# GStreamer/gst-plugins-rs

Hardware: AMD Instinct MI355X
Metric: 4K RGBA frames/sec through hsvfilter+colorlut at 1 GPU; % HBM roofline (higher is better)
Workload: dtype u8

## Files before the change

gst-plugins-rs_amd/csrc/autopick.hpp:

```cpp
#pragma once
#include <cstddef>

namespace mi355 {

constexpr unsigned kProbeMin = 64, kProbeMax = 1024;
constexpr double kDecisive = 2.0;
constexpr double kRegimeChange = 1.25;

struct AutoPolicy {
  unsigned calls = 0, since_probe = 0, probe_period = kProbeMin;
  bool table = false;
  double t_compute = 0.0, t_table = 0.0;
  size_t vec = 0;
  int pending_kind = -1;
  size_t pending_vec = 0;
  unsigned pending_call = 0;
  bool pending_probe = false, pending_discard = false;
  unsigned learn = 0;
  bool probe_second = false;
  bool table_unavailable = false;
  double hysteresis = 0.03;
  double hysteresis_back = -1.0;
  bool smooth = false;
  bool last_probe = false;
// ... 55 lines not shown
    D.discard = (A.learn & 1) == 0;
    D.probe = true;
    if (A.pending_kind < 0) A.learn++;
  } else {
    D.kind = A.table ? 1 : 0;
    bool warming = false;
    if (A.probe_second) {
      A.probe_second = false;
      D.kind ^= 1;
      D.probe = true;
    } else if (++A.since_probe >= A.probe_period && A.pending_kind < 0) {
      A.since_probe = 0;
      A.probe_second = true;
      D.kind ^= 1;
      warming = true;
    }
    if (warming) { A.calls++; return D; }
  }
  D.measure = A.pending_kind < 0 && (D.probe || (A.calls % auto_sample_every(n_vec)) == 0);
  A.calls++;
  return D;
}

inline void auto_sampled(AutoPolicy &A, const AutoDecision &D, size_t n_vec) {
  A.pending_kind = D.kind;
  A.pending_call = A.calls;
  A.pending_vec = n_vec;
  A.pending_probe = D.probe && A.t_compute > 0.0 && A.t_table > 0.0;
  A.pending_discard = D.discard;
}

inline void auto_give_up_table(AutoPolicy &A) {
  A.table_unavailable = true;
  A.learn = 4;
  A.table = false;
}

}
```

gst-plugins-rs_amd/csrc/colorlut_kernels.hip:

```cpp
#include "internal.hpp"
#include "hsv_device.hpp"
#include "exact_math.hpp"

#include <cmath>
#include <cstring>
#include <map>
#include <memory>
#include <mutex>
#include <vector>

namespace mi355 {

struct LutK {
  float scale[3];
  float offset[3];
  int size;
};


__device__ __forceinline__ uint32_t floor_idx(float x, uint32_t max_idx) {
  const float f = floorf(x);
  uint32_t i = (f > 0.0f) ? ((f >= 4294967040.0f) ? 0xffffffffu : (uint32_t)f) : 0u;
  return i < max_idx ? i : max_idx;
}
// ... 825 lines not shown
  __shared__ uint32_t s_strip[4][512];
  s_spread[threadIdx.x] = spread3(threadIdx.x);
  __syncthreads();
  auto index = [&](uint32_t p) -> uint32_t { return s_spread[p & 0xffu] | (s_spread[(p >> 8) & 0xffu] << 1) | (s_spread[(p >> 16) & 0xffu] << 2); };
  const unsigned wave = threadIdx.x >> 6, lane = threadIdx.x & 63;
  uint32_t *x = s_strip[wave];
  const unsigned frame = blockIdx.x / tiles_per_frame, t = blockIdx.x - frame * tiles_per_frame;
  const u32x4_t *s4 = (const u32x4_t *)srcs.p[frame];
  u32x4_t *d4 = (u32x4_t *)dsts.p[frame];
  auto wave_sync = [] {
    __builtin_amdgcn_fence(__ATOMIC_ACQ_REL, "wavefront");
    __builtin_amdgcn_wave_barrier();
  };
  constexpr unsigned RPL = 64 / TW4;
  const unsigned sub = lane / TW4, g = lane % TW4;
  const unsigned tx = t % n_cols, ty = t / n_cols;
  const unsigned col = tx * TW4 + g;
  const unsigned r0 = ty * (8 * RPL) + wave * (2 * RPL) + sub, r1 = r0 + RPL;
  const bool ok0 = col < w4 && r0 < rows, ok1 = col < w4 && r1 < rows;
  const size_t i0 = (size_t)r0 * w4 + col, i1 = (size_t)r1 * w4 + col;
  u32x4_t p = {0, 0, 0, 0}, q = {0, 0, 0, 0};
  if (ok0) p = __builtin_nontemporal_load(s4 + i0);
  if (ok1) q = __builtin_nontemporal_load(s4 + i1);
  *(u32x4_t *)(x + lane * 4) = p;
  *(u32x4_t *)(x + 256 + lane * 4) = q;
  wave_sync();
  uint32_t px[8], o[8];
#pragma unroll
  for (int j = 0; j < 8; j++) px[j] = x[j * 64 + lane];
#pragma unroll
  for (int j = 0; j < 8; j++) o[j] = table[index(px[j])];
#pragma unroll
  for (int j = 0; j < 8; j++) x[j * 64 + lane] = (o[j] & 0x00ffffffu) | (px[j] & 0xff000000u);
  wave_sync();
  const u32x4_t r0v = *(u32x4_t *)(x + lane * 4), r1v = *(u32x4_t *)(x + 256 + lane * 4);
  if (ok0) __builtin_nontemporal_store(r0v, d4 + i0);
  if (ok1) __builtin_nontemporal_store(r1v, d4 + i1);
}

void shared_table_release(mi355_ctx *ctx, std::shared_ptr<void> *ref);
void lut_release(mi355_ctx *ctx) {
  for (int i = 0; i < 2; i++) {
    shared_table_release(ctx, &ctx->lut.table_ref[i]);
    if (ctx->lut.pick[i].ev0) (void)hipEventDestroy(ctx->lut.pick[i].ev0);
    if (ctx->lut.pick[i].ev1) (void)hipEventDestroy(ctx->lut.pick[i].ev1);
  }
// ... 713 lines not shown
  MultiFramePtrs s{}, d{};
  for (int f = 0; f < n_frames; f++) {
    if (!srcs[f] || !dsts[f] || (uintptr_t)srcs[f] % 16 != 0 || (uintptr_t)dsts[f] % 16 != 0) return MI355_ERR_UNSUPPORTED;
    s.p[f] = srcs[f];
    d.p[f] = dsts[f];
  }
  const unsigned w4 = (unsigned)width / 4;
  if (from_hbm && ctx->lut_variant == 0 && window_multi_applicable(ctx, w4, (size_t)height, n_frames)) {
    ctx->lut.last_kernel = "colorlut_window_kernel";
    return launch_window_table_multi(ctx, stream, table, srcs, dsts, n_frames, w4, (size_t)height);
  }
  ctx->lut.last_kernel = "colorlut_table_tiled_multi_kernel";
  const unsigned pad64 = (w4 + 63) / 64 * 64 - w4, pad32 = (w4 + 31) / 32 * 32 - w4;
  const unsigned tw4 = pad64 <= pad32 ? 64 : 32;
  const unsigned n_cols = (w4 + tw4 - 1) / tw4, rpb = 8 * (64 / tw4);
  const size_t tiles_per_frame = (size_t)n_cols * (((size_t)height + rpb - 1) / rpb);
  const size_t grid = tiles_per_frame * (size_t)n_frames;
  if (grid >= (1u << 31)) return MI355_ERR_UNSUPPORTED;
  if (tw4 == 64) hipLaunchKernelGGL((colorlut_table_tiled_multi_kernel<64>), dim3((unsigned)grid), dim3(256), 0, stream, s, d, w4, (unsigned)height, n_cols, (unsigned)tiles_per_frame, table);
  else hipLaunchKernelGGL((colorlut_table_tiled_multi_kernel<32>), dim3((unsigned)grid), dim3(256), 0, stream, s, d, w4, (unsigned)height, n_cols, (unsigned)tiles_per_frame, table);
  return check_hip(ctx, hipGetLastError(), "colorlut multi-frame table kernel launch");
}

void hsv_table_release(mi355_ctx *ctx) {
  HsvTable &T = ctx->hsv_table;
  shared_table_release(ctx, &T.table_ref);
  if (T.pick.ev0) (void)hipEventDestroy(T.pick.ev0);
  if (T.pick.ev1) (void)hipEventDestroy(T.pick.ev1);
  T = HsvTable{};
}

static int hsv_table_ensure(mi355_ctx *ctx, const PixFmt &fmt, const mi355_hsv_settings &hs) {
  HsvTable &T = ctx->hsv_table;
  if (T.valid && T.bgr == fmt.bgr && same_hs(T.hs, hs)) return MI355_OK;
  T.valid = false;
  T.d_table = nullptr;
  std::string key("H");
  key.push_back((char)('0' + fmt.bgr));
  key.append((const char *)&hs, sizeof(hs));
  int rc = shared_table_acquire(ctx, key, &T.table_ref, &T.d_table, [&](uint32_t *tab) {
    hipLaunchKernelGGL(table_domain_kernel, dim3(kTableEntries / 256), dim3(256), 0, ctx->stream, tab, 1);
    return launch_hsvfilter_compute(ctx, (uint8_t *)tab, 1, 0, 4096, 4096, 4096 * 4, fmt, hs);
  });
  if (rc) { T.table_ref.reset(); T.d_table = nullptr; return rc; }
  T.valid = true;
  T.bgr = fmt.bgr;
// ... 67 lines not shown
```

gst-plugins-rs_amd/csrc/ctx.hip:

```cpp
#include "internal.hpp"
#include <mutex>

#include <cstdio>
#include <cstring>

namespace mi355 {

bool pixfmt_of(int format, PixFmt *out) {
  switch (format) {
    case MI355_FMT_RGBX: *out = {4, 0, 0, 0}; return true;
    case MI355_FMT_RGBA: *out = {4, 0, 0, 1}; return true;
    case MI355_FMT_XRGB: *out = {4, 1, 0, 0}; return true;
    case MI355_FMT_ARGB: *out = {4, 1, 0, 1}; return true;
    case MI355_FMT_BGRX: *out = {4, 0, 1, 0}; return true;
    case MI355_FMT_BGRA: *out = {4, 0, 1, 1}; return true;
    case MI355_FMT_XBGR: *out = {4, 1, 1, 0}; return true;
    case MI355_FMT_ABGR: *out = {4, 1, 1, 1}; return true;
    case MI355_FMT_RGB: *out = {3, 0, 0, 0}; return true;
    case MI355_FMT_BGR: *out = {3, 0, 1, 0}; return true;
    default: return false;
  }
}

int set_error(mi355_ctx *ctx, int status, const std::string &msg) {
// ... 61 lines not shown
}

const char *mi355_status_string(int status) {
  switch (status) {
    case MI355_OK: return "ok";
    case MI355_ERR_INVALID_ARG: return "invalid argument";
    case MI355_ERR_NO_DEVICE: return "no usable gfx950 device";
    case MI355_ERR_HIP: return "HIP runtime error";
    case MI355_ERR_NOT_CONFIGURED: return "element not configured";
    case MI355_ERR_OUT_OF_MEMORY: return "out of device memory";
    case MI355_ERR_UNSUPPORTED: return "unsupported";
    case MI355_ERR_TIMEOUT: return "timeout";
    default: return "unknown status";
  }
}

}

namespace mi355 {
namespace {
struct Written { uintptr_t lo = 0, hi = 0; };
std::mutex g_written_mu;
Written g_written[16][2];
constexpr size_t kOnDieBytes = (size_t)320 << 20;
}

void note_written(int device, const void *p, size_t bytes) {
  if (device < 0 || device >= 16 || !p || !bytes) return;
  std::lock_guard<std::mutex> lk(g_written_mu);
  g_written[device][1] = g_written[device][0];
  g_written[device][0].lo = (uintptr_t)p;
  g_written[device][0].hi = (uintptr_t)p + bytes;
}

void forget_written(int device, const void *p, size_t bytes) {
  if (device < 0 || device >= 16 || !p || !bytes) return;
  std::lock_guard<std::mutex> lk(g_written_mu);
  for (Written &w : g_written[device])
    if (w.hi > w.lo && (uintptr_t)p < w.hi && (uintptr_t)p + bytes > w.lo) w = Written{};
}

bool recently_written(int device, const void *p, size_t bytes) {
  if (device < 0 || device >= 16 || !p || !bytes || bytes > kOnDieBytes) return false;
  std::lock_guard<std::mutex> lk(g_written_mu);
  for (const Written &w : g_written[device])
    if (w.hi > w.lo && (uintptr_t)p >= w.lo && (uintptr_t)p + bytes <= w.hi && w.hi - w.lo <= kOnDieBytes) return true;
  return false;
// ... 81 lines not shown

int mi355_ctx_synchronize(mi355_ctx *ctx) {
  REQUIRE_CTX(ctx);
  BIND_DEVICE(ctx);
  return check_hip(ctx, hipStreamSynchronize(ctx->stream), "hipStreamSynchronize");
}

int mi355_ctx_set_flag(mi355_ctx *ctx, int flag, int value) {
  REQUIRE_CTX(ctx);
  if (flag == MI355_FLAG_FORCE_GENERIC) { ctx->force_generic = value != 0; return MI355_OK; }
  if (flag == MI355_FLAG_LUT_STAGGER && value >= 0 && value <= 4096) { ctx->lut_stagger = value; return MI355_OK; }
  if (flag == MI355_FLAG_LUT_VARIANT && value >= 0 && value <= 9) { ctx->lut_variant = value; return MI355_OK; }
  if (flag == MI355_FLAG_BRICK_TILES_PER_RUN && value >= 0 && value <= 4096) { ctx->brick_tiles_per_run = value; return MI355_OK; }
  if (flag == MI355_FLAG_BRICK_FOLD_AXIS && value >= 0 && value <= 2) { ctx->brick_fold_axis = value; return MI355_OK; }
  if (flag == MI355_FLAG_DSSIM_TRANSLUCENT && (value == 0 || value == 1)) { ctx->dssim_translucent = value; return MI355_OK; }
  if (flag == MI355_FLAG_DSSIM_FAST && (value == 0 || value == 1)) { ctx->dssim_fast = value; return MI355_OK; }
  if (flag == MI355_FLAG_BRICK_PRIO && value >= 0 && value <= 3) { ctx->brick_prio = value; return MI355_OK; }
  if (flag == MI355_FLAG_BRICK_SETS && (value == 0 || value == 32 || value == 48 || value == 64 || value == 512)) { ctx->brick_sets = value; return MI355_OK; }
  if (flag == MI355_FLAG_HSV_TABLE && value >= 0 && value <= 3) { ctx->hsv_table_mode = value; return MI355_OK; }
  if (flag == MI355_FLAG_FUSED_VARIANT && value >= 0 && value <= 1) { ctx->fused_variant = value; return MI355_OK; }
  if (flag == MI355_FLAG_HSV_BLOCKS_PER_CU && value >= 1 && value <= 4096) { ctx->hsv_blocks_per_cu = value; return MI355_OK; }
  if (flag == MI355_FLAG_HRTF_METHOD && value >= 0 && value <= 2) { ctx->hrtf_method = value; return MI355_OK; }
  if (flag == MI355_FLAG_BLOCKHASH_ANY_SIZE && (value == 0 || value == 1)) { ctx->blockhash_any_size = value; return MI355_OK; }
  if (flag == MI355_FLAG_HSV_NT && (value == 0 || value == 1)) { ctx->hsv_nt = value; return MI355_OK; }
  if (flag == MI355_FLAG_WINDOW_ORDER && (value == 0 || value == 1)) { ctx->window_order = value; return MI355_OK; }
  if (flag == MI355_FLAG_WINDOW_STATS && (value == 0 || value == 1)) { ctx->window_stats_on = value != 0; return MI355_OK; }
  if (flag == MI355_FLAG_WINDOW_MIN_STEPS && value >= 0 && value <= 4096) { ctx->window_min_steps = value; return MI355_OK; }
  return set_error(ctx, MI355_ERR_INVALID_ARG, "unknown flag");
}

void *mi355_device_alloc(mi355_ctx *ctx, size_t bytes) {
  if (!ctx) return nullptr;
  if (hipSetDevice(ctx->device) != hipSuccess) return nullptr;
  void *p = nullptr;
  if (check_hip(ctx, hipMalloc(&p, bytes ? bytes : 16), "hipMalloc")) return nullptr;
  return p;
}

int mi355_device_free(mi355_ctx *ctx, void *dptr) {
  REQUIRE_CTX(ctx);
  BIND_DEVICE(ctx);
  return check_hip(ctx, hipFree(dptr), "hipFree");
}

int mi355_memcpy_h2d(mi355_ctx *ctx, void *dptr, const void *host, size_t bytes) {
  REQUIRE_CTX(ctx);
  BIND_DEVICE(ctx);
// ... 592 lines not shown
}

int mi355_issue_streams_round(mi355_ctx *const *ctxs, int n_streams, uint8_t *const *d_src, uint8_t *const *d_dst, int width, int height, int stride,
                              int format, const mi355_hsv_settings *settings) {
  if (!ctxs || !d_src || !d_dst || !settings || n_streams < 0) return MI355_ERR_INVALID_ARG;
  const size_t pitch = (size_t)stride * (size_t)(height > 0 ? height : 0);
  for (int i = 0; i < n_streams; i++) {
    int rc = mi355_hsvfilter_frames_device(ctxs[i], d_src[i], 1, pitch, width, height, stride, format, settings);
    if (rc) return rc;
    rc = mi355_colorlut_frames_device(ctxs[i], d_src[i], pitch, stride, d_dst[i], pitch, stride, 1, width, height, format);
    if (rc) return rc;
  }
  return MI355_OK;
}

int mi355_hsv_colorlut_chain_batches_device(mi355_ctx *ctx, uint8_t *const *d_src, uint8_t *const *d_dst, int n_batches, int n_frames, size_t frame_pitch,
                                            int stride, int width, int height, int format, const mi355_hsv_settings *settings, int lanes) {
  REQUIRE_CTX(ctx);
  if (!d_src || !d_dst || !settings || n_batches < 0 || lanes < 1 || lanes > 2) return set_error(ctx, MI355_ERR_INVALID_ARG, "chain batches: bad argument");
  BIND_DEVICE(ctx);
  int rc = MI355_OK;
  for (int k = 0; k < n_batches && !rc; k++) {
    if (!d_src[k] || !d_dst[k]) { rc = set_error(ctx, MI355_ERR_INVALID_ARG, "chain batches: null batch"); break; }
    rc = mi355_hsvfilter_frames_device(ctx, d_src[k], n_frames, frame_pitch, width, height, stride, format, settings);
    if (!rc) rc = mi355_colorlut_frames_device(ctx, d_src[k], frame_pitch, stride, d_dst[k], frame_pitch, stride, n_frames, width, height, format);
  }
  return rc;
}

int mi355_dssim_compare_frames_device(mi355_ctx *ctx, const mi355_dssim_image *original, const uint8_t *const *d_frames, int n_frames, int stride,
                                      int width, int height, int format, double *dssim) {
  REQUIRE_CTX(ctx);
  int channels = 0;
  int rc = dssim_channels(ctx, format, &channels);
  if (rc) return rc;
  if (!original || !d_frames || !dssim || n_frames < 0 || width <= 0 || height <= 0 || (size_t)stride < (size_t)width * channels)
    return set_error(ctx, MI355_ERR_INVALID_ARG, "dssim: bad frames");
  for (int f = 0; f < n_frames; f++)
    if (!d_frames[f]) return set_error(ctx, MI355_ERR_INVALID_ARG, "dssim: null frame");
  if (n_frames == 0) return MI355_OK;
  BIND_DEVICE(ctx);
  return dssim_compare_frames(ctx, original, d_frames, n_frames, stride, width, height, channels, dssim);
}

int mi355_dssim_compare_frames(mi355_ctx *ctx, const mi355_dssim_image *original, const uint8_t *const *frames, int n_frames, int stride, int width,
                               int height, int format, double *dssim) {
// ... 199 lines not shown
```

gst-plugins-rs_amd/csrc/group.hip:

```cpp
#include "internal.hpp"

#include <chrono>
#include <condition_variable>
#include <algorithm>
#include <cstring>
#include <deque>
#include <mutex>
#include <unordered_map>
#include <vector>

using namespace mi355;

namespace {

struct Desc {
  mi355_ctx *ctx;
  uint8_t *src, *dst;
  int width, height, stride, format;
  mi355_hsv_settings hs;
  const uint32_t *table;
  std::shared_ptr<void> table_ref;
  bool batchable;
  bool fused;
  uint64_t ticket;
// ... 743 lines not shown
    if (!lk.owns_lock()) lk.lock();
    reap.swap(g->dead_refs);
    lk.unlock();
  }
};

void retire_front(mi355_group *g) {
  Batch &b = g->batches.front();
  for (uint64_t t : b.tickets) g->where.erase(t);
  g->events.push_back(b.done);
  if (b.table_ref) g->dead_refs.push_back(std::move(b.table_ref));
  g->batches.pop_front();
}

void retire_done(mi355_group *g) {
  while (!g->batches.empty() && g->batches.front().waiters == 0) {
    if (hipEventQuery(g->batches.front().done) != hipSuccess) { (void)hipGetLastError(); break; }
    retire_front(g);
  }
}

bool same_class(const Desc &a, const Desc &b) {
  return a.batchable && b.batchable && a.fused == b.fused && a.width == b.width && a.height == b.height && a.stride == b.stride && a.format == b.format && a.table == b.table &&
         std::memcmp(&a.hs, &b.hs, sizeof(a.hs)) == 0 && a.ctx->force_generic == b.ctx->force_generic;
}

int flush_locked(mi355_group *g, uint64_t until = 0) {
  bool reached = false;
  while (!g->pending.empty() && !reached) {
    std::vector<Desc> take, keep;
    std::vector<mi355_ctx *> blocked;
    const Desc first = g->pending.front();
    for (const Desc &d : g->pending) {
      bool stream_blocked = false;
      for (mi355_ctx *c : blocked) stream_blocked |= c == d.ctx;
      const bool fits = take.empty() || (!stream_blocked && (int)take.size() < g->max_batch && same_class(first, d));
      if (fits) take.push_back(d);
      else keep.push_back(d);
      if (!stream_blocked) blocked.push_back(d.ctx);
    }
    g->pending.swap(keep);
    PixFmt fmt;
    (void)pixfmt_of(first.format, &fmt);
    hipEvent_t done = take_event(g);
    if (!done) return fail(g, MI355_ERR_HIP, "hipEventCreate");
    int rc = MI355_OK;
    if (first.batchable) {
      uint8_t *srcs[kMultiFrames], *dsts[kMultiFrames];
      for (size_t i = 0; i < take.size(); i++) {
        srcs[i] = take[i].src;
        dsts[i] = take[i].dst;
        if (take[i].ready && hipStreamWaitEvent(g->stream, take[i].ready, 0) != hipSuccess) rc = MI355_ERR_HIP;
      }
      if (!rc && !first.fused) rc = launch_hsvfilter_multi(first.ctx, g->stream, srcs, (int)take.size(), first.width, first.height, fmt, first.hs);
      if (!rc) rc = launch_colorlut_multi(first.ctx, g->stream, first.table, srcs, dsts, (int)take.size(), first.width, first.height, first.fused);
      if (!rc && hipEventRecord(done, g->stream) != hipSuccess) rc = MI355_ERR_HIP;
      g->n_batched_launch_pairs++;
    } else {
      const Desc &d = take[0];
      const size_t pitch = (size_t)d.stride * (size_t)d.height;
      if (!g->batches.empty() && hipStreamWaitEvent(d.ctx->stream, g->batches.back().done, 0) != hipSuccess) rc = MI355_ERR_HIP;
      if (!rc && d.fused) rc = launch_hsv_colorlut(d.ctx, d.src, pitch, d.stride, d.dst, pitch, d.stride, 1, d.width, d.height, d.hs);
      if (!rc && !d.fused) rc = launch_hsvfilter(d.ctx, d.src, 1, pitch, d.width, d.height, d.stride, fmt, d.hs);
      if (!rc && !d.fused) rc = launch_colorlut(d.ctx, d.src, pitch, d.stride, d.dst, pitch, d.stride, 1, d.width, d.height, d.format);
      if (!rc && hipEventRecord(done, d.ctx->stream) != hipSuccess) rc = MI355_ERR_HIP;
      if (!rc && hipStreamWaitEvent(g->stream, done, 0) != hipSuccess) rc = MI355_ERR_HIP;
      if (rc && rc != MI355_ERR_HIP) g->last_error = d.ctx->last_error;
      g->n_single++;
    }
    for (const Desc &d : take)
      if (d.ready) g->events.push_back(d.ready);
    if (rc) {
      (void)hipGetLastError();
      g->events.push_back(done);
      if (g->failed.size() > 65536) g->failed.clear();
      for (const Desc &d : take) g->failed[d.ticket] = rc;
      if (g->last_error.empty()) g->last_error = "group launch failed";
      return rc;
// ... 575 lines not shown
```

gst-plugins-rs_amd/csrc/hsv_device.hpp:

```cpp
#pragma once
#include "internal.hpp"
#include "exact_math.hpp"

namespace mi355 {

struct HsvK {
  float hue_shift, sat_mul, sat_off, val_mul, val_off;
};


template <bool FAST>
__device__ __forceinline__ void hsv_from_rgb(float r8, float g8, float b8, float &hue, float &sat,
                                             float &val) {
  if constexpr (FAST) {
    const float r = div255_u8(r8), g = div255_u8(g8), b = div255_u8(b8);
    const float value = fmaxf(fmaxf(r, g), b);
    const float minv = fminf(fminf(r, g), b);
    const float chroma = value - minv;
    const bool is_r = (r == value);
    const bool is_g = (g == value);
    const float na = is_r ? g : (is_g ? b : r);
    const float nb = is_r ? b : (is_g ? r : g);
    const float add = is_r ? 0.0f : (is_g ? 2.0f : 4.0f);
    const float q = div_rcp_refine(na - nb, fmaxf(chroma, 1e-30f));
    float h = 60.0f * (add + q);
// ... 288 lines not shown
    r = (r >= 360.0f) ? r - 360.0f : r;
    return __builtin_copysignf(r, t);
  }
  return fmodf(t, 360.0f);
}
template <int RPOS, int GPOS, int BPOS, int NPOS>
__device__ __forceinline__ void hsvfilter_px2_generic(uint32_t &p0, uint32_t &p1, const HsvK &k, const HsvLds *lds) {
  f2 h2, sat, value;
  hsv_from_rgb_pair_fast<RPOS, GPOS, BPOS, 1>(p0, p1, h2, sat, value, lds);
  uint32_t *px[2] = {&p0, &p1};
#pragma unroll
  for (int j = 0; j < 2; j++) {
    float h = hsv_fmod360_any((j ? h2.y : h2.x) + k.hue_shift);
    if (h < 0.0f) h += 360.0f;
    const float s = fminf(fmaxf(k.sat_mul * (j ? sat.y : sat.x) + k.sat_off, 0.0f), 1.0f);
    const float v = fminf(fmaxf(k.val_mul * (j ? value.y : value.x) + k.val_off, 0.0f), 1.0f);
    uint32_t r, g, b;
    hsv_to_rgb_generic(h, s, v, r, g, b);
    const uint32_t keep = *px[j] & (0xffu << (8 * NPOS));
    *px[j] = keep | (r << (8 * RPOS)) | (g << (8 * GPOS)) | (b << (8 * BPOS));
  }
}

inline int hsv_variant_for(const mi355_hsv_settings &s, bool force_generic, bool allow_wide = false) {
  const float a = fabsf(s.hue_shift);
  const bool narrow = (s.hue_shift == 0.0f) || (a >= 1e-30f && a <= 360.0f);
  const bool wide = allow_wide && a > 360.0f && a <= 4194304.0f;
  if (!(narrow || wide) || force_generic) return -1;
  const bool sv_ident = s.saturation_mul == 1.0f && s.saturation_off == 0.0f && s.value_mul == 1.0f && s.value_off == 0.0f;
  if (wide) return 8 | (s.hue_shift < 0.0f ? 1 : 0) | (sv_ident ? 4 : 0);
  const int shift = s.hue_shift == 0.0f ? HSV_SHIFT_ZERO : (s.hue_shift > 0.0f ? HSV_SHIFT_POS : HSV_SHIFT_NEG);
  return shift | (sv_ident ? 4 : 0);
}

}
```

gst-plugins-rs_amd/csrc/hsv_kernels.hip:

```cpp
#include "internal.hpp"
#include "exact_math.hpp"
#include "hsv_device.hpp"

namespace mi355 {


template <int VARIANT, int RPOS, int GPOS, int BPOS, int NPOS>
__device__ __forceinline__ void hsvfilter_quad(uint32_t &a, uint32_t &b, uint32_t &c, uint32_t &d, const HsvK &k, const HsvLds *lds) {
  if constexpr (VARIANT >= 0) {
    hsvfilter_px2_lds<RPOS, GPOS, BPOS, NPOS, hsv_shift_of(VARIANT), hsv_sv_ident_of(VARIANT)>(a, b, k, lds);
    hsvfilter_px2_lds<RPOS, GPOS, BPOS, NPOS, hsv_shift_of(VARIANT), hsv_sv_ident_of(VARIANT)>(c, d, k, lds);
  } else {
    hsvfilter_px2_generic<RPOS, GPOS, BPOS, NPOS>(a, b, k, lds);
    hsvfilter_px2_generic<RPOS, GPOS, BPOS, NPOS>(c, d, k, lds);
  }
}

template <int VARIANT, int FIRST, bool BGR>
__global__ __launch_bounds__(256) void hsvfilter_flat_kernel(uint4 *__restrict__ data, size_t n_vec,
                                                             HsvK k, int nt) {
  constexpr int RPOS = FIRST + (BGR ? 2 : 0), GPOS = FIRST + 1, BPOS = FIRST + (BGR ? 0 : 2);
  constexpr int NPOS = FIRST == 0 ? 3 : 0;
  __shared__ HsvLds lds;
  hsv_lds_fill<RPOS, GPOS, BPOS, NPOS>(&lds);
  __syncthreads();
  const size_t stride = (size_t)gridDim.x * blockDim.x;
  if (nt) {
    typedef uint32_t u32x4_t __attribute__((ext_vector_type(4)));
    u32x4_t *d4 = (u32x4_t *)data;
    for (size_t i = (size_t)blockIdx.x * blockDim.x + threadIdx.x; i < n_vec; i += stride) {
      const u32x4_t v = __builtin_nontemporal_load(d4 + i);
      uint4 p = {v.x, v.y, v.z, v.w};
      hsvfilter_quad<VARIANT, RPOS, GPOS, BPOS, NPOS>(p.x, p.y, p.z, p.w, k, &lds);
      const u32x4_t o = {p.x, p.y, p.z, p.w};
      __builtin_nontemporal_store(o, d4 + i);
    }
    return;
  }
  for (size_t i = (size_t)blockIdx.x * blockDim.x + threadIdx.x; i < n_vec; i += stride) {
// ... 162 lines not shown
    const size_t r = i - f * per_frame;
    const size_t row = r / (size_t)width;
    const size_t col = r - row * (size_t)width;
    uint8_t *px = data + f * frame_pitch + row * (size_t)stride + col * (size_t)pixel_stride + first;
    const uint32_t c0 = px[0], c1 = px[1], c2 = px[2];
    const uint32_t p = bgr ? (c2 | (c1 << 8) | (c0 << 16)) : (c0 | (c1 << 8) | (c2 << 16));
    const uint32_t o = hsvfilter_px<FAST, 0, 1, 2, 3>(p, k, sel_tab);
    const uint8_t orr = (uint8_t)(o & 0xff), og = (uint8_t)((o >> 8) & 0xff), ob = (uint8_t)((o >> 16) & 0xff);
    px[0] = bgr ? ob : orr;
    px[1] = og;
    px[2] = bgr ? orr : ob;
  }
}

static int grid_for(mi355_ctx *ctx, size_t work_items, int block, int blocks_per_cu) {
  size_t blocks = (work_items + (size_t)block - 1) / (size_t)block;
  size_t cap = (size_t)ctx->n_cu * (size_t)blocks_per_cu;
  if (blocks > cap) blocks = cap;
  if (blocks < 1) blocks = 1;
  return (int)blocks;
}


template <class F>
static void with_variant(int variant, F &&f) {
  switch (variant) {
    case -1: f(std::integral_constant<int, -1>{}); break;
    case 0: f(std::integral_constant<int, 0>{}); break;
    case 1: f(std::integral_constant<int, 1>{}); break;
    case 2: f(std::integral_constant<int, 2>{}); break;
    case 4: f(std::integral_constant<int, 4>{}); break;
    case 5: f(std::integral_constant<int, 5>{}); break;
    case 6: f(std::integral_constant<int, 6>{}); break;
    case 8: f(std::integral_constant<int, 8>{}); break;
    case 9: f(std::integral_constant<int, 9>{}); break;
    case 12: f(std::integral_constant<int, 12>{}); break;
    default: f(std::integral_constant<int, 13>{}); break;
  }
}

template <class F>
static void with_flag(bool on, F &&f) {
  if (on) f(std::true_type{});
  else f(std::false_type{});
}

template <class F>
static void with_byte_order(int first, int bgr, F &&f) {
  if (first == 0 && !bgr) f(std::integral_constant<int, 0>{}, std::false_type{});
  else if (first == 0 && bgr) f(std::integral_constant<int, 0>{}, std::true_type{});
  else if (first == 1 && !bgr) f(std::integral_constant<int, 1>{}, std::false_type{});
  else f(std::integral_constant<int, 1>{}, std::true_type{});
}

static void launch_flat(mi355_ctx *ctx, int variant, uint4 *d, size_t n_vec, const HsvK &k, int first, int bgr, int grid) {
  const int nt = ctx->hsv_nt;
  with_variant(variant, [&](auto V) { with_byte_order(first, bgr, [&](auto FIRST, auto BGR) {
    hipLaunchKernelGGL((hsvfilter_flat_kernel<V, FIRST, BGR>), dim3(grid), dim3(256), 0, ctx->stream, d, n_vec, k, nt);
  }); });
}

static void launch_strided(mi355_ctx *ctx, int variant, uint8_t *d, int n_frames, size_t frame_pitch, int width, int height, int stride, const HsvK &k,
// ... 658 lines not shown
```

gst-plugins-rs_amd/csrc/internal.hpp:

```cpp
#pragma once
#include <hip/hip_runtime.h>
#include <cstddef>
#include <cstdint>
#include <cstring>
#include <memory>
#include <string>
#include <vector>
#include "../../include/mi355fx.h"

#include "autopick.hpp"
#include "colorlut_brick.hpp"
#include "colorlut_window.hpp"

namespace mi355 {

struct AutoPick : AutoPolicy {
  hipEvent_t ev0 = nullptr, ev1 = nullptr;
};

constexpr unsigned kStableCalls = 8;
struct Settled {
  mi355_hsv_settings hs{};
  int bgr = 0;
  unsigned stable = 0;
// ... 81 lines not shown
  unsigned long long n_h2d = 0, n_d2h = 0;
  bool force_generic = false;
  int fused_variant = 0;
  int lut_variant = 0;
  int hsv_table_mode = 0;
  mi355::HsvTable hsv_table;
  int lut_stagger = 0;
  int brick_tiles_per_run = 0;
  int brick_fold_axis = 2;
  hipEvent_t host_copy_ev = nullptr;
  int dssim_translucent = 0;
  int dssim_fast = 0;
  int brick_prio = 3;
  int brick_sets = 0;
  int hrtf_method = 0;
  int window_min_steps = mi355::kWindowMinStepsPerBlock;
  int window_order = 1;
  bool window_stats_on = false;
  unsigned long long *d_window_counters = nullptr;
  int blockhash_any_size = 0;
  int hsv_nt = 0;
  mi355_hsv_settings group_fused_hs{};
  unsigned group_fused_stable = 0;
  int hsv_blocks_per_cu = 64;
  std::string last_error;
};

namespace mi355 {

constexpr int kMultiFrames = 16;
struct MultiFramePtrs { uint8_t *p[kMultiFrames]; };

struct PixFmt {
  int pixel_stride;
  int first;
  int bgr;
  int has_alpha;
};
bool pixfmt_of(int format, PixFmt *out);

int set_error(mi355_ctx *ctx, int status, const std::string &msg);
void note_written(int device, const void *p, size_t bytes);
bool recently_written(int device, const void *p, size_t bytes);
void forget_written(int device, const void *p, size_t bytes);
int check_hip(mi355_ctx *ctx, hipError_t e, const char *what);

template <typename T, bool PINNED>
struct GrowBuf {
  T *p = nullptr;
  size_t n = 0;
  GrowBuf() = default;
  GrowBuf(const GrowBuf &) = delete;
  GrowBuf &operator=(const GrowBuf &) = delete;
  ~GrowBuf() { release(); }
  void release() {
    if (p) (void)(PINNED ? hipHostFree(p) : hipFree(p));
    p = nullptr;
    n = 0;
  }
  hipError_t reserve(size_t want, bool *fresh = nullptr) {
    if (n >= want && p) return hipSuccess;
    release();
    if (fresh) *fresh = true;
    const hipError_t e = PINNED ? hipHostMalloc((void **)&p, want * sizeof(T), hipHostMallocDefault) : hipMalloc((void **)&p, want * sizeof(T));
// ... 1 lines not shown
      (void)hipGetLastError();
      p = nullptr;
      return e;
    }
    n = want;
    return hipSuccess;
  }
};
template <typename T> using DeviceBuf = GrowBuf<T, false>;
template <typename T> using PinnedBuf = GrowBuf<T, true>;

int launch_hsvfilter(mi355_ctx *ctx, uint8_t *d_data, int n_frames, size_t frame_pitch, int width,
                     int height, int stride, const PixFmt &fmt, const mi355_hsv_settings &s);
int launch_hsvfilter_compute(mi355_ctx *ctx, uint8_t *d_data, int n_frames, size_t frame_pitch, int width,
                     int height, int stride, const PixFmt &fmt, const mi355_hsv_settings &s);
void hsv_table_release(mi355_ctx *ctx);
bool hsvfilter_multi_applicable(const uint8_t *const *frames, int n_frames, int width, int height, int stride, const PixFmt &fmt);
int launch_hsvfilter_multi(mi355_ctx *ctx, hipStream_t stream, uint8_t *const *frames, int n_frames, int width, int height, const PixFmt &fmt,
                           const mi355_hsv_settings &s);
int colorlut_multi_table(mi355_ctx *ctx, const uint32_t **table_out);
int colorlut_multi_fused_table(mi355_ctx *ctx, const mi355_hsv_settings *hs, const uint32_t **table_out);
int launch_colorlut_multi(mi355_ctx *ctx, hipStream_t stream, const uint32_t *table, uint8_t *const *srcs, uint8_t *const *dsts, int n_frames, int width,
                          int height, bool from_hbm = false);
int launch_hsvdetect(mi355_ctx *ctx, const uint8_t *d_src, size_t src_pitch, int src_stride,
                     const PixFmt &sfmt, uint8_t *d_dst, size_t dst_pitch, int dst_stride,
                     int dst_alpha_first, int dst_bgr, int n_frames, int width, int height,
                     const mi355_hsvdetect_settings &s);
int launch_colorlut(mi355_ctx *ctx, const uint8_t *d_src, size_t src_pitch, int src_stride,
                    uint8_t *d_dst, size_t dst_pitch, int dst_stride, int n_frames, int width,
                    int height, int format);
int launch_hsv_colorlut(mi355_ctx *ctx, const uint8_t *d_src, size_t src_pitch, int src_stride,
                        uint8_t *d_dst, size_t dst_pitch, int dst_stride, int n_frames, int width,
                        int height, const mi355_hsv_settings &hs);
bool table_variant(int lut_variant);
int lut_upload(mi355_ctx *ctx, int is3d, size_t size, const float *table, const float scale[3],
               const float offset[3]);
void lut_release(mi355_ctx *ctx);
int echo_setup(mi355_ctx *ctx, int n_streams, size_t ring_len);
void echo_release(mi355_ctx *ctx);
int launch_echo_batch(mi355_ctx *ctx, void *d_data, size_t stream_stride, size_t n, int is_f64, const size_t *delay, const double *intensity,
                      const double *feedback);
int launch_echo(mi355_ctx *ctx, void *d_data, size_t n, int is_f64, size_t delay, double intensity,
                double feedback);
int ebur128_setup(mi355_ctx *ctx, unsigned channels, unsigned rate, unsigned mode, const int *channel_class);
int ebur128_setup_batch(mi355_ctx *ctx, unsigned n_streams, unsigned channels, unsigned rate, unsigned mode, const int *channel_class);
int ebur128_add_frames_batch(mi355_ctx *ctx, const void *data, size_t frames, int fmt, int device_data);
// ... 223 lines not shown
```

gst-plugins-rs_amd/mi355fx/__init__.py:

```python
import ctypes as C
import os

import numpy as np

_HERE = os.path.dirname(os.path.abspath(__file__))
PKG_ROOT = os.path.dirname(_HERE)
LIB_PATH = os.environ.get("MI355FX_LIB") or os.path.join(PKG_ROOT, "libmi355fx.so")
HEADER_PATH = os.path.join(os.path.dirname(PKG_ROOT), "include", "mi355fx.h")

FMT = {"RGBx": 0, "xRGB": 1, "BGRx": 2, "xBGR": 3, "RGBA": 4, "ARGB": 5, "BGRA": 6, "ABGR": 7,
       "RGB": 8, "BGR": 9, "RGBA64_LE": 10, "RGBA64_BE": 11}
FMT_LAYOUT = {"RGBx": (4, 0, 0), "RGBA": (4, 0, 0), "RGB": (3, 0, 0), "xRGB": (4, 1, 0), "ARGB": (4, 1, 0),
              "BGRx": (4, 0, 1), "BGRA": (4, 0, 1), "BGR": (3, 0, 1), "xBGR": (4, 1, 1), "ABGR": (4, 1, 1)}

OK, ERR_INVALID_ARG, ERR_NO_DEVICE, ERR_HIP, ERR_NOT_CONFIGURED, ERR_OOM, ERR_UNSUPPORTED, ERR_TIMEOUT = 0, -1, -2, -3, -4, -5, -6, -7
FLAG_FORCE_GENERIC = 1
FLAG_HSV_BLOCKS_PER_CU = 2
FLAG_FUSED_VARIANT = 3
FLAG_LUT_VARIANT = 4
FLAG_LUT_STAGGER = 5
FLAG_HSV_TABLE = 6
FLAG_BRICK_TILES_PER_RUN = 7
FLAG_BRICK_SETS = 8
FLAG_BRICK_PRIO = 9
FLAG_BRICK_FOLD_AXIS = 10
FLAG_DSSIM_TRANSLUCENT = 11
FLAG_HRTF_METHOD = 12
FLAG_WINDOW_MIN_STEPS = 13
FLAG_HSV_NT = 14
FLAG_BLOCKHASH_ANY_SIZE = 15
FLAG_WINDOW_ORDER = 17
FLAG_WINDOW_STATS = 18
FLAG_DSSIM_FAST = 19
HSVDETECT_SET_MAX = 32
HSVFILTER_SET_MAX = 32
YOLODEC_SET_MAX = 32
MIXER_FRAME_TILE = 64


class HsvSettings(C.Structure):
    _fields_ = [("hue_shift", C.c_float), ("saturation_mul", C.c_float), ("saturation_off", C.c_float),
                ("value_mul", C.c_float), ("value_off", C.c_float)]


class HsvFilterPlanFrame(C.Structure):
    _fields_ = [("address", C.c_uint64), ("width", C.c_int32), ("height", C.c_int32), ("stride", C.c_int32), ("format", C.c_int32),
                ("settings", HsvSettings), ("force_generic", C.c_int32)]


class HsvFilterPlanOut(C.Structure):
    _fields_ = [("set", C.c_int32), ("launch", C.c_int32), ("variant", C.c_int32), ("first_block", C.c_uint32), ("blocks", C.c_uint32),
                ("reserved", C.c_uint32), ("units", C.c_uint64)]


class AgingRadioSettings(C.Structure):
    _fields_ = [("white_noise_ampl", C.c_float), ("clicks_prob", C.c_float), ("bits_to_quantize", C.c_float),
# ... 1910 lines not shown
```

include/mi355fx.h:

```cpp
#ifndef MI355FX_H
#define MI355FX_H

#include <stddef.h>
#include <stdint.h>

#ifdef __cplusplus
extern "C" {
#endif

#define MI355FX_ABI_VERSION 1

typedef enum mi355_status {
  MI355_OK = 0,
  MI355_ERR_INVALID_ARG = -1,
  MI355_ERR_NO_DEVICE = -2,
  MI355_ERR_HIP = -3,
  MI355_ERR_NOT_CONFIGURED = -4,
  MI355_ERR_OUT_OF_MEMORY = -5,
  MI355_ERR_UNSUPPORTED = -6,
  MI355_ERR_TIMEOUT = -7
} mi355_status;

typedef enum mi355_video_format {
  MI355_FMT_RGBX = 0,
// ... 18 lines not shown
mi355_ctx *mi355_ctx_create(int device, int *status);
void mi355_ctx_destroy(mi355_ctx *ctx);
const char *mi355_ctx_last_error(const mi355_ctx *ctx);
const char *mi355_status_string(int status);
void *mi355_ctx_stream(mi355_ctx *ctx);
int mi355_ctx_set_stream(mi355_ctx *ctx, void *hip_stream);
int mi355_ctx_synchronize(mi355_ctx *ctx);

typedef enum mi355_flag {
  MI355_FLAG_FORCE_GENERIC = 1,
  MI355_FLAG_HSV_BLOCKS_PER_CU = 2,
  MI355_FLAG_LUT_VARIANT = 4,
  MI355_FLAG_HSV_TABLE = 6,
  MI355_FLAG_LUT_STAGGER = 5,
  MI355_FLAG_FUSED_VARIANT = 3,
  MI355_FLAG_BRICK_TILES_PER_RUN = 7,
  MI355_FLAG_DSSIM_TRANSLUCENT = 11,
  MI355_FLAG_DSSIM_FAST = 19,
  MI355_FLAG_BRICK_FOLD_AXIS = 10,
  MI355_FLAG_BRICK_PRIO = 9,
  MI355_FLAG_HRTF_METHOD = 12,
  MI355_FLAG_BLOCKHASH_ANY_SIZE = 15,
  MI355_FLAG_HSV_NT = 14,
  MI355_FLAG_WINDOW_ORDER = 17,
  MI355_FLAG_WINDOW_STATS = 18,
  MI355_FLAG_WINDOW_MIN_STEPS = 13,
  MI355_FLAG_BRICK_SETS = 8
} mi355_flag;
int mi355_ctx_set_flag(mi355_ctx *ctx, int flag, int value);

void *mi355_device_alloc(mi355_ctx *ctx, size_t bytes);
int mi355_device_free(mi355_ctx *ctx, void *dptr);
int mi355_memcpy_h2d(mi355_ctx *ctx, void *dptr, const void *host, size_t bytes);
int mi355_memcpy_d2h(mi355_ctx *ctx, void *host, const void *dptr, size_t bytes);

typedef struct mi355_hsv_settings {
  float hue_shift;
  float saturation_mul;
  float saturation_off;
  float value_mul;
  float value_off;
} mi355_hsv_settings;

int mi355_hsvfilter_frame_ip(mi355_ctx *ctx, uint8_t *data, size_t data_len, int width, int stride,
                             int format, const mi355_hsv_settings *settings);
int mi355_hsvfilter_frames_device(mi355_ctx *ctx, uint8_t *d_data, int n_frames, size_t frame_pitch,
// ... 537 lines not shown
```

Measured before the change: 44900.

## Fuse hsvfilter and colorlut into one chain kernel for RGBA batches

Adds a single kernel that loads each tile once, applies the HSV filter in registers, writes the HSV result back to the source, then runs the LUT table lookup through LDS and stores to the destination. With chain_launch at its default of 0, the chain-batch path uses it when the autopicker would select the plain table path on this call, or for LUT variants 5 and 9. The group path uses it only when the flag is 2. This removes one kernel launch and a full re-read of the intermediate frame from HBM. The cost is extra gating logic and autopicker bookkeeping, and the fused kernel bypasses the window kernel in some size regimes.

```diff
diff --git a/gst-plugins-rs_amd/csrc/autopick.hpp b/gst-plugins-rs_amd/csrc/autopick.hpp
--- a/gst-plugins-rs_amd/csrc/autopick.hpp
+++ b/gst-plugins-rs_amd/csrc/autopick.hpp
@@ -101,6 +101,18 @@
   return D;
 }
 
+inline bool auto_plain_table_next(const AutoPolicy &A, size_t n_vec) {
+  if (A.table_unavailable || A.learn < 4 || !A.table || A.probe_second) return false;
+  if (A.vec && (n_vec > 2 * A.vec || 2 * n_vec < A.vec)) return false;
+  if (A.since_probe + 1 >= A.probe_period && A.pending_kind < 0) return false;
+  if (A.pending_kind < 0 && (A.calls % auto_sample_every(n_vec)) == 0) return false;
+  return true;
+}
+inline void auto_pass(AutoPolicy &A) {
+  A.since_probe++;
+  A.calls++;
+}
+
 inline void auto_sampled(AutoPolicy &A, const AutoDecision &D, size_t n_vec) {
   A.pending_kind = D.kind;
   A.pending_call = A.calls;
diff --git a/gst-plugins-rs_amd/csrc/colorlut_kernels.hip b/gst-plugins-rs_amd/csrc/colorlut_kernels.hip
--- a/gst-plugins-rs_amd/csrc/colorlut_kernels.hip
+++ b/gst-plugins-rs_amd/csrc/colorlut_kernels.hip
@@ -871,6 +871,59 @@
   u32x4_t p = {0, 0, 0, 0}, q = {0, 0, 0, 0};
   if (ok0) p = __builtin_nontemporal_load(s4 + i0);
   if (ok1) q = __builtin_nontemporal_load(s4 + i1);
+  *(u32x4_t *)(x + lane * 4) = p;
+  *(u32x4_t *)(x + 256 + lane * 4) = q;
+  wave_sync();
+  uint32_t px[8], o[8];
+#pragma unroll
+  for (int j = 0; j < 8; j++) px[j] = x[j * 64 + lane];
+#pragma unroll
+  for (int j = 0; j < 8; j++) o[j] = table[index(px[j])];
+#pragma unroll
+  for (int j = 0; j < 8; j++) x[j * 64 + lane] = (o[j] & 0x00ffffffu) | (px[j] & 0xff000000u);
+  wave_sync();
+  const u32x4_t r0v = *(u32x4_t *)(x + lane * 4), r1v = *(u32x4_t *)(x + 256 + lane * 4);
+  if (ok0) __builtin_nontemporal_store(r0v, d4 + i0);
+  if (ok1) __builtin_nontemporal_store(r1v, d4 + i1);
+}
+
+template <int VARIANT>
+__global__ __launch_bounds__(256) void hsv_colorlut_chain_multi_kernel(MultiFramePtrs srcs, MultiFramePtrs dsts, unsigned w4, unsigned rows, unsigned n_cols,
+                                                                       unsigned tiles_per_frame, const uint32_t *__restrict__ table, HsvK k) {
+  constexpr unsigned TW4 = 64;
+  __shared__ HsvLds s_hsv;
+  __shared__ uint32_t s_spread[256];
+  __shared__ uint32_t s_strip[4][512];
+  hsv_lds_fill<0, 1, 2, 3>(&s_hsv);
+  s_spread[threadIdx.x] = spread3(threadIdx.x);
+  __syncthreads();
+  auto index = [&](uint32_t p) -> uint32_t { return s_spread[p & 0xffu] | (s_spread[(p >> 8) & 0xffu] << 1) | (s_spread[(p >> 16) & 0xffu] << 2); };
+  const unsigned wave = threadIdx.x >> 6, lane = threadIdx.x & 63;
+  uint32_t *x = s_strip[wave];
+  const unsigned frame = blockIdx.x / tiles_per_frame, t = blockIdx.x - frame * tiles_per_frame;
+  u32x4_t *s4 = (u32x4_t *)srcs.p[frame];
+  u32x4_t *d4 = (u32x4_t *)dsts.p[frame];
+  auto wave_sync = [] {
+    __builtin_amdgcn_fence(__ATOMIC_ACQ_REL, "wavefront");
+    __builtin_amdgcn_wave_barrier();
+  };
+  constexpr unsigned RPL = 64 / TW4;
+  const unsigned sub = lane / TW4, g = lane % TW4;
+  const unsigned tx = t % n_cols, ty = t / n_cols;
+  const unsigned col = tx * TW4 + g;
+  const unsigned r0 = ty * (8 * RPL) + wave * (2 * RPL) + sub, r1 = r0 + RPL;
+  const bool ok0 = col < w4 && r0 < rows, ok1 = col < w4 && r1 < rows;
+  const size_t i0 = (size_t)r0 * w4 + col, i1 = (size_t)r1 * w4 + col;
+  u32x4_t p = {0, 0, 0, 0}, q = {0, 0, 0, 0};
+  if (ok0) p = __builtin_nontemporal_load(s4 + i0);
+  if (ok1) q = __builtin_nontemporal_load(s4 + i1);
+  uint32_t a[8] = {p.x, p.y, p.z, p.w, q.x, q.y, q.z, q.w};
+  hsvfilter_quad<VARIANT, 0, 1, 2, 3>(a[0], a[1], a[2], a[3], k, &s_hsv);
+  hsvfilter_quad<VARIANT, 0, 1, 2, 3>(a[4], a[5], a[6], a[7], k, &s_hsv);
+  p = u32x4_t{a[0], a[1], a[2], a[3]};
+  q = u32x4_t{a[4], a[5], a[6], a[7]};
+  if (ok0) __builtin_nontemporal_store(p, s4 + i0);
+  if (ok1) __builtin_nontemporal_store(q, s4 + i1);
   *(u32x4_t *)(x + lane * 4) = p;
   *(u32x4_t *)(x + 256 + lane * 4) = q;
   wave_sync();
@@ -1630,6 +1683,98 @@
   return check_hip(ctx, hipGetLastError(), "colorlut multi-frame table kernel launch");
 }
 
+bool chain_launch_wanted(const mi355_ctx *ctx) { return ctx->chain_launch == 2; }
+
+static bool ranges_disjoint(const uint8_t *const *p, int n, size_t bytes) {
+  for (int i = 0; i < n; i++)
+    for (int j = i + 1; j < n; j++)
+      if ((uintptr_t)p[i] < (uintptr_t)p[j] + bytes && (uintptr_t)p[j] < (uintptr_t)p[i] + bytes) return false;
+  return true;
+}
+
+static bool chain_geometry_ok(uint8_t *const *srcs, uint8_t *const *dsts, int n_frames, int width, int height, size_t *grid_out, size_t *tiles_per_frame_out) {
+  if (n_frames < 1 || n_frames > kMultiFrames || width % 4 != 0 || width < 128 || height <= 0) return false;
+  const uint8_t *all[2 * kMultiFrames];
+  for (int f = 0; f < n_frames; f++) {
+    if (!srcs[f] || !dsts[f] || (uintptr_t)srcs[f] % 16 != 0 || (uintptr_t)dsts[f] % 16 != 0) return false;
+    all[2 * f] = srcs[f];
+    all[2 * f + 1] = dsts[f];
+  }
+  if (!ranges_disjoint(all, 2 * n_frames, (size_t)width * 4 * (size_t)height)) return false;
+  const size_t n_cols = ((size_t)width / 4 + 63) / 64;
+  *tiles_per_frame_out = n_cols * (((size_t)height + 7) / 8);
+  *grid_out = *tiles_per_frame_out * (size_t)n_frames;
+  return *grid_out < (1u << 31);
+}
+
+static int launch_chain_kernel(mi355_ctx *ctx, hipStream_t stream, const uint32_t *table, uint8_t *const *srcs, uint8_t *const *dsts, int n_frames, int width, int height,
+                               size_t grid, size_t tiles_per_frame, const mi355_hsv_settings &hs) {
+  MultiFramePtrs s{}, d{};
+  for (int f = 0; f < n_frames; f++) { s.p[f] = srcs[f]; d.p[f] = dsts[f]; }
+  const HsvK k{hs.hue_shift, hs.saturation_mul, hs.saturation_off, hs.value_mul, hs.value_off};
+  const int variant = hsv_variant_for(hs, ctx->force_generic, true);
+  const unsigned w4 = (unsigned)width / 4, n_cols = (w4 + 63) / 64;
+  ctx->lut.last_kernel = "hsv_colorlut_chain_multi_kernel";
+  with_variant(variant, [&](auto V) {
+    hipLaunchKernelGGL((hsv_colorlut_chain_multi_kernel<V>), dim3((unsigned)grid), dim3(256), 0, stream, s, d, w4, (unsigned)height, n_cols, (unsigned)tiles_per_frame, table, k);
+  });
+  return check_hip(ctx, hipGetLastError(), "hsvfilter ! colorlut chain kernel launch");
+}
+
+int launch_chain_multi(mi355_ctx *ctx, hipStream_t stream, const uint32_t *table, uint8_t *const *srcs, uint8_t *const *dsts, int n_frames, int width,
+                       int height, const PixFmt &fmt, const mi355_hsv_settings &hs) {
+  size_t grid = 0, tiles_per_frame = 0;
+  const bool rgba_class = fmt.pixel_stride == 4 && fmt.first == 0 && !fmt.bgr;
+  if (chain_launch_wanted(ctx) && table && rgba_class && ctx->lut_variant == 0 && chain_geometry_ok(srcs, dsts, n_frames, width, height, &grid, &tiles_per_frame)) {
+    const int rc = launch_chain_kernel(ctx, stream, table, srcs, dsts, n_frames, width, height, grid, tiles_per_frame, hs);
+    if (rc) return rc;
+    const size_t bytes = (size_t)width * 4 * (size_t)height;
+    for (int f = 0; f < n_frames; f++) note_written(ctx->device, srcs[f], bytes);
+    for (int f = 0; f < n_frames; f++) note_written(ctx->device, dsts[f], bytes);
+    return MI355_OK;
+  }
+  const int rc = launch_hsvfilter_multi(ctx, stream, srcs, n_frames, width, height, fmt, hs);
+  return rc ? rc : launch_colorlut_multi(ctx, stream, table, srcs, dsts, n_frames, width, height, false);
+}
+
+int launch_chain_frames(mi355_ctx *ctx, uint8_t *d_src, uint8_t *d_dst, int n_frames, size_t frame_pitch, int stride, int width, int height, int format,
+                        const mi355_hsv_settings &hs, bool *took) {
+  *took = false;
+  LutDevice &L = ctx->lut;
+  if (ctx->chain_launch == 1 || !L.loaded || format != MI355_FMT_RGBA || ctx->force_generic || ctx->hsv_nt) return MI355_OK;
+  if (n_frames < 1 || n_frames > kMultiFrames || width <= 0 || height <= 0) return MI355_OK;
+  const size_t frame_bytes = (size_t)width * 4 * (size_t)height;
+  if ((size_t)stride != (size_t)width * 4 || (n_frames > 1 && frame_pitch != frame_bytes)) return MI355_OK;
+  if (!(ctx->hsv_table_mode == 3 || (ctx->hsv_table_mode == 0 && hsv_variant_for(hs, false, true) >= 0))) return MI355_OK;
+  const int v = ctx->lut_variant;
+  if (v != 0 && v != 5 && v != 9) return MI355_OK;
+  uint8_t *srcs[kMultiFrames], *dsts[kMultiFrames];
+  for (int f = 0; f < n_frames; f++) { srcs[f] = d_src + (size_t)f * frame_bytes; dsts[f] = d_dst + (size_t)f * frame_bytes; }
+  size_t grid = 0, tiles_per_frame = 0;
+  if (!chain_geometry_ok(srcs, dsts, n_frames, width, height, &grid, &tiles_per_frame)) return MI355_OK;
+  const size_t rows = (size_t)n_frames * (size_t)height, n_vec = frame_bytes * (size_t)n_frames / 16;
+  if (rows >= (1u << 30)) return MI355_OK;
+  const unsigned w4 = (unsigned)width / 4;
+  if (v != 5 && frame_bytes * (size_t)n_frames > kOnDieBytes && window_applicable(ctx, w4, w4, rows)) return MI355_OK;
+  AutoPick &A = L.pick[0];
+  if (v == 0) {
+    if (n_vec < kAutoMinVec || !L.table_ref[0] || !L.d_table[0] || L.table_morton[0] != 1) return MI355_OK;
+    auto_harvest(A);
+    if (!auto_plain_table_next(A, n_vec)) return MI355_OK;
+  } else if (table_ensure(ctx, 0, 1, nullptr)) {
+    (void)hipGetLastError();
+    return MI355_OK;
+  }
+  const int rc = launch_chain_kernel(ctx, ctx->stream, L.d_table[0], srcs, dsts, n_frames, width, height, grid, tiles_per_frame, hs);
+  if (rc) return rc;
+  if (v == 0) auto_pass(A);
+  note_written(ctx->device, d_src, frame_bytes * (size_t)n_frames);
+  note_written(ctx->device, d_dst, frame_bytes * (size_t)n_frames);
+  L.last_sub[0] = 0;
+  *took = true;
+  return MI355_OK;
+}
+
 void hsv_table_release(mi355_ctx *ctx) {
   HsvTable &T = ctx->hsv_table;
   shared_table_release(ctx, &T.table_ref);
diff --git a/gst-plugins-rs_amd/csrc/ctx.hip b/gst-plugins-rs_amd/csrc/ctx.hip
--- a/gst-plugins-rs_amd/csrc/ctx.hip
+++ b/gst-plugins-rs_amd/csrc/ctx.hip
@@ -107,7 +107,6 @@
 struct Written { uintptr_t lo = 0, hi = 0; };
 std::mutex g_written_mu;
 Written g_written[16][2];
-constexpr size_t kOnDieBytes = (size_t)320 << 20;
 }
 
 void note_written(int device, const void *p, size_t bytes) {
@@ -235,7 +234,8 @@
   if (flag == MI355_FLAG_HSV_BLOCKS_PER_CU && value >= 1 && value <= 4096) { ctx->hsv_blocks_per_cu = value; return MI355_OK; }
   if (flag == MI355_FLAG_HRTF_METHOD && value >= 0 && value <= 2) { ctx->hrtf_method = value; return MI355_OK; }
   if (flag == MI355_FLAG_BLOCKHASH_ANY_SIZE && (value == 0 || value == 1)) { ctx->blockhash_any_size = value; return MI355_OK; }
-  if (flag == MI355_FLAG_HSV_NT && (value == 0 || value == 1)) { ctx->hsv_nt = value; return MI355_OK; }
+  if (flag == MI355_FLAG_CHAIN_LAUNCH && value >= 0 && value <= 2) { ctx->chain_launch = value; return MI355_OK; }
+  if (flag == MI355_FLAG_HSV_NT &&(value == 0 || value == 1)) { ctx->hsv_nt = value; return MI355_OK; }
   if (flag == MI355_FLAG_WINDOW_ORDER && (value == 0 || value == 1)) { ctx->window_order = value; return MI355_OK; }
   if (flag == MI355_FLAG_WINDOW_STATS && (value == 0 || value == 1)) { ctx->window_stats_on = value != 0; return MI355_OK; }
   if (flag == MI355_FLAG_WINDOW_MIN_STEPS && value >= 0 && value <= 4096) { ctx->window_min_steps = value; return MI355_OK; }
@@ -874,6 +874,9 @@
   int rc = MI355_OK;
   for (int k = 0; k < n_batches && !rc; k++) {
     if (!d_src[k] || !d_dst[k]) { rc = set_error(ctx, MI355_ERR_INVALID_ARG, "chain batches: null batch"); break; }
+    bool took = false;
+    rc = launch_chain_frames(ctx, d_src[k], d_dst[k], n_frames, frame_pitch, stride, width, height, format, *settings, &took);
+    if (rc || took) continue;
     rc = mi355_hsvfilter_frames_device(ctx, d_src[k], n_frames, frame_pitch, width, height, stride, format, settings);
     if (!rc) rc = mi355_colorlut_frames_device(ctx, d_src[k], frame_pitch, stride, d_dst[k], frame_pitch, stride, n_frames, width, height, format);
   }
diff --git a/gst-plugins-rs_amd/csrc/group.hip b/gst-plugins-rs_amd/csrc/group.hip
--- a/gst-plugins-rs_amd/csrc/group.hip
+++ b/gst-plugins-rs_amd/csrc/group.hip
@@ -789,7 +789,8 @@
 
 bool same_class(const Desc &a, const Desc &b) {
   return a.batchable && b.batchable && a.fused == b.fused && a.width == b.width && a.height == b.height && a.stride == b.stride && a.format == b.format && a.table == b.table &&
-         std::memcmp(&a.hs, &b.hs, sizeof(a.hs)) == 0 && a.ctx->force_generic == b.ctx->force_generic;
+         std::memcmp(&a.hs, &b.hs, sizeof(a.hs)) == 0 && a.ctx->force_generic == b.ctx->force_generic &&
+         chain_launch_wanted(a.ctx) == chain_launch_wanted(b.ctx);
 }
 
 int flush_locked(mi355_group *g, uint64_t until = 0) {
@@ -819,8 +820,8 @@
         dsts[i] = take[i].dst;
         if (take[i].ready && hipStreamWaitEvent(g->stream, take[i].ready, 0) != hipSuccess) rc = MI355_ERR_HIP;
       }
-      if (!rc && !first.fused) rc = launch_hsvfilter_multi(first.ctx, g->stream, srcs, (int)take.size(), first.width, first.height, fmt, first.hs);
-      if (!rc) rc = launch_colorlut_multi(first.ctx, g->stream, first.table, srcs, dsts, (int)take.size(), first.width, first.height, first.fused);
+      if (!rc && first.fused) rc = launch_colorlut_multi(first.ctx, g->stream, first.table, srcs, dsts, (int)take.size(), first.width, first.height, true);
+      else if (!rc) rc = launch_chain_multi(first.ctx, g->stream, first.table, srcs, dsts, (int)take.size(), first.width, first.height, fmt, first.hs);
       if (!rc && hipEventRecord(done, g->stream) != hipSuccess) rc = MI355_ERR_HIP;
       g->n_batched_launch_pairs++;
     } else {
diff --git a/gst-plugins-rs_amd/csrc/hsv_device.hpp b/gst-plugins-rs_amd/csrc/hsv_device.hpp
--- a/gst-plugins-rs_amd/csrc/hsv_device.hpp
+++ b/gst-plugins-rs_amd/csrc/hsv_device.hpp
@@ -1,6 +1,8 @@
 #pragma once
 #include "internal.hpp"
 #include "exact_math.hpp"
+
+#include <type_traits>
 
 namespace mi355 {
 
@@ -335,6 +337,17 @@
   }
 }
 
+template <int VARIANT, int RPOS, int GPOS, int BPOS, int NPOS>
+__device__ __forceinline__ void hsvfilter_quad(uint32_t &a, uint32_t &b, uint32_t &c, uint32_t &d, const HsvK &k, const HsvLds *lds) {
+  if constexpr (VARIANT >= 0) {
+    hsvfilter_px2_lds<RPOS, GPOS, BPOS, NPOS, hsv_shift_of(VARIANT), hsv_sv_ident_of(VARIANT)>(a, b, k, lds);
+    hsvfilter_px2_lds<RPOS, GPOS, BPOS, NPOS, hsv_shift_of(VARIANT), hsv_sv_ident_of(VARIANT)>(c, d, k, lds);
+  } else {
+    hsvfilter_px2_generic<RPOS, GPOS, BPOS, NPOS>(a, b, k, lds);
+    hsvfilter_px2_generic<RPOS, GPOS, BPOS, NPOS>(c, d, k, lds);
+  }
+}
+
 inline int hsv_variant_for(const mi355_hsv_settings &s, bool force_generic, bool allow_wide = false) {
   const float a = fabsf(s.hue_shift);
   const bool narrow = (s.hue_shift == 0.0f) || (a >= 1e-30f && a <= 360.0f);
@@ -346,4 +359,21 @@
   return shift | (sv_ident ? 4 : 0);
 }
 
-}
+template <class F>
+inline void with_variant(int variant, F &&f) {
+  switch (variant) {
+    case -1: f(std::integral_constant<int, -1>{}); break;
+    case 0: f(std::integral_constant<int, 0>{}); break;
+    case 1: f(std::integral_constant<int, 1>{}); break;
+    case 2: f(std::integral_constant<int, 2>{}); break;
+    case 4: f(std::integral_constant<int, 4>{}); break;
+    case 5: f(std::integral_constant<int, 5>{}); break;
+    case 6: f(std::integral_constant<int, 6>{}); break;
+    case 8: f(std::integral_constant<int, 8>{}); break;
+    case 9: f(std::integral_constant<int, 9>{}); break;
+    case 12: f(std::integral_constant<int, 12>{}); break;
+    default: f(std::integral_constant<int, 13>{}); break;
+  }
+}
+
+}
diff --git a/gst-plugins-rs_amd/csrc/hsv_kernels.hip b/gst-plugins-rs_amd/csrc/hsv_kernels.hip
--- a/gst-plugins-rs_amd/csrc/hsv_kernels.hip
+++ b/gst-plugins-rs_amd/csrc/hsv_kernels.hip
@@ -5,16 +5,6 @@
 namespace mi355 {
 
 
-template <int VARIANT, int RPOS, int GPOS, int BPOS, int NPOS>
-__device__ __forceinline__ void hsvfilter_quad(uint32_t &a, uint32_t &b, uint32_t &c, uint32_t &d, const HsvK &k, const HsvLds *lds) {
-  if constexpr (VARIANT >= 0) {
-    hsvfilter_px2_lds<RPOS, GPOS, BPOS, NPOS, hsv_shift_of(VARIANT), hsv_sv_ident_of(VARIANT)>(a, b, k, lds);
-    hsvfilter_px2_lds<RPOS, GPOS, BPOS, NPOS, hsv_shift_of(VARIANT), hsv_sv_ident_of(VARIANT)>(c, d, k, lds);
-  } else {
-    hsvfilter_px2_generic<RPOS, GPOS, BPOS, NPOS>(a, b, k, lds);
-    hsvfilter_px2_generic<RPOS, GPOS, BPOS, NPOS>(c, d, k, lds);
-  }
-}
 
 template <int VARIANT, int FIRST, bool BGR>
 __global__ __launch_bounds__(256) void hsvfilter_flat_kernel(uint4 *__restrict__ data, size_t n_vec,
@@ -223,22 +213,6 @@
 }
 
 
-template <class F>
-static void with_variant(int variant, F &&f) {
-  switch (variant) {
-    case -1: f(std::integral_constant<int, -1>{}); break;
-    case 0: f(std::integral_constant<int, 0>{}); break;
-    case 1: f(std::integral_constant<int, 1>{}); break;
-    case 2: f(std::integral_constant<int, 2>{}); break;
-    case 4: f(std::integral_constant<int, 4>{}); break;
-    case 5: f(std::integral_constant<int, 5>{}); break;
-    case 6: f(std::integral_constant<int, 6>{}); break;
-    case 8: f(std::integral_constant<int, 8>{}); break;
-    case 9: f(std::integral_constant<int, 9>{}); break;
-    case 12: f(std::integral_constant<int, 12>{}); break;
-    default: f(std::integral_constant<int, 13>{}); break;
-  }
-}
 
 template <class F>
 static void with_flag(bool on, F &&f) {
diff --git a/gst-plugins-rs_amd/csrc/internal.hpp b/gst-plugins-rs_amd/csrc/internal.hpp
--- a/gst-plugins-rs_amd/csrc/internal.hpp
+++ b/gst-plugins-rs_amd/csrc/internal.hpp
@@ -127,6 +127,7 @@
   int hsv_nt = 0;
   mi355_hsv_settings group_fused_hs{};
   unsigned group_fused_stable = 0;
+  int chain_launch = 0;
   int hsv_blocks_per_cu = 64;
   std::string last_error;
 };
@@ -145,6 +146,7 @@
 bool pixfmt_of(int format, PixFmt *out);
 
 int set_error(mi355_ctx *ctx, int status, const std::string &msg);
+constexpr size_t kOnDieBytes = (size_t)320 << 20;
 void note_written(int device, const void *p, size_t bytes);
 bool recently_written(int device, const void *p, size_t bytes);
 void forget_written(int device, const void *p, size_t bytes);
@@ -192,6 +194,11 @@
 int colorlut_multi_fused_table(mi355_ctx *ctx, const mi355_hsv_settings *hs, const uint32_t **table_out);
 int launch_colorlut_multi(mi355_ctx *ctx, hipStream_t stream, const uint32_t *table, uint8_t *const *srcs, uint8_t *const *dsts, int n_frames, int width,
                           int height, bool from_hbm = false);
+bool chain_launch_wanted(const mi355_ctx *ctx);
+int launch_chain_multi(mi355_ctx *ctx, hipStream_t stream, const uint32_t *table, uint8_t *const *srcs, uint8_t *const *dsts, int n_frames, int width,
+                       int height, const PixFmt &fmt, const mi355_hsv_settings &hs);
+int launch_chain_frames(mi355_ctx *ctx, uint8_t *d_src, uint8_t *d_dst, int n_frames, size_t frame_pitch, int stride, int width, int height, int format,
+                        const mi355_hsv_settings &hs, bool *took);
 int launch_hsvdetect(mi355_ctx *ctx, const uint8_t *d_src, size_t src_pitch, int src_stride,
                      const PixFmt &sfmt, uint8_t *d_dst, size_t dst_pitch, int dst_stride,
                      int dst_alpha_first, int dst_bgr, int n_frames, int width, int height,
diff --git a/gst-plugins-rs_amd/mi355fx/__init__.py b/gst-plugins-rs_amd/mi355fx/__init__.py
--- a/gst-plugins-rs_amd/mi355fx/__init__.py
+++ b/gst-plugins-rs_amd/mi355fx/__init__.py
@@ -32,6 +32,7 @@
 FLAG_WINDOW_ORDER = 17
 FLAG_WINDOW_STATS = 18
 FLAG_DSSIM_FAST = 19
+FLAG_CHAIN_LAUNCH = 20
 HSVDETECT_SET_MAX = 32
 HSVFILTER_SET_MAX = 32
 YOLODEC_SET_MAX = 32
diff --git a/include/mi355fx.h b/include/mi355fx.h
--- a/include/mi355fx.h
+++ b/include/mi355fx.h
@@ -64,6 +64,7 @@
   MI355_FLAG_HRTF_METHOD = 12,
   MI355_FLAG_BLOCKHASH_ANY_SIZE = 15,
   MI355_FLAG_HSV_NT = 14,
+  MI355_FLAG_CHAIN_LAUNCH = 20,
   MI355_FLAG_WINDOW_ORDER = 17,
   MI355_FLAG_WINDOW_STATS = 18,
   MI355_FLAG_WINDOW_MIN_STEPS = 13,
```

New measurement: 44860. No clear change (-0.1%).
